# qurAI-amsterdam/SuperResolution_aniso_MRI

Measured on AMD Instinct MI355X. Metric: training slices/sec (ae_combined, 160x160, latent=128), higher is better.
Workload: dtype f32; 1 GPU; ACDC synthetic 12x(3x1x160x160) triplets, ae_combined latent=128 depth=32 scales=2, MSE synthesis loss (BASELINE configs[1]); global_batch_triplets=12, parallelism=dp1, init=reference Initializer, seed 892372, random weights, launch=captured HIP graph replay

## Files before the change

### superresolution_aniso_mri_amd/csrc/aesr_api.hip

```cpp
#include <stdarg.h>
#include <stdio.h>
#include <stdlib.h>
#include <string.h>

#include <map>
#include <mutex>
#include <tuple>

#include "../../include/aesr_hip.h"
#include "../../include/aesr_hip_dataprep.h"
#include "aesr_kernels.h"

static thread_local char g_err[512] = "";
void aesr_set_error(const char* fmt, ...) {
    va_list ap;
    va_start(ap, fmt);
    vsnprintf(g_err, sizeof(g_err), fmt, ap);
    va_end(ap);
}

static void cout_padding(int Cout, int* CoutP, int* NB) {
    if (Cout <= 16) { *CoutP = 16; *NB = 1; }
    else if (Cout <= 32) { *CoutP = 32; *NB = 2; }
    else { *CoutP = round_up(Cout, 64); *NB = 4; }
}

static bool conv_dims_ok(int N, int H, int W, int Cin, int Cout) {
    if (N < 1 || H < 1 || W < 1 || Cin < 1 || Cout < 1) return false;
    if (N > (1 << 24) || H > (1 << 15) || W > (1 << 15) || Cin > (1 << 15) || Cout > (1 << 15)) return false;
    const unsigned long long px = (unsigned long long)N * (unsigned)(H + 2) * (unsigned)(W + 2);
    return px * (unsigned long long)(Cin > Cout ? Cin : Cout) < 0x1C000000ull;
}
#define AESR_CHECK_DIMS(who, N, H, W, Cin, Cout)                                                                                            \
    do {                                                                                                                                    \
        if (!conv_dims_ok(N, H, W, Cin, Cout)) {                                                                                            \
            aesr_set_error("%s: %d x %d x %d with %d -> %d channels is empty or beyond the kernels' 32-bit element offsets (469M elements)", who, N, H, \
                           W, Cin, Cout);                                                                                                   \
            return AESR_ERR_UNSUPPORTED;                                                                                                    \
        }                                                                                                                                   \
    } while (0)

struct ConvPlan { int TI, TH, TW, NB, MBW, CinP, CoutP, NT, ksplit; };
static std::mutex g_plan_mu;

static std::map<std::tuple<int, int, int, int, int, int>, ConvPlan> g_conv_plans;

static ConvPlan plan_conv(int N, int Ho, int Wo, int Cin, int Cout, int KS) {
    std::lock_guard<std::mutex> lk(g_plan_mu);
    const auto key = std::make_tuple(N, Ho, Wo, Cin, Cout, KS);
    auto it = g_conv_plans.find(key);
    if (it != g_conv_plans.end()) return it->second;
    ConvPlan p;
    cout_padding(Cout, &p.CoutP, &p.NB);
    p.CinP = round_up(Cin, 16);
    p.MBW = (p.NB == 4) ? 2 : 4;
    const int ncout = p.CoutP / (16 * p.NB);
    int force_nt = 0;
    if (const char* e = getenv("AESR_IGEMM_NT")) force_nt = atoi(e);
    double best = 1e300;
    p.TI = 1; p.TH = 1; p.TW = 1; p.NT = 512;
// ... 58 lines not shown
}

struct WinoPlan { int TI, THt, TWt, CinP, CoutP; double cost; };
static std::map<std::tuple<int, int, int, int, int>, WinoPlan> g_wino_plans;

static WinoPlan plan_wino(int N, int H, int W, int Cin, int Cout) {
    std::lock_guard<std::mutex> lk(g_plan_mu);
    const auto key = std::make_tuple(N, H, W, Cin, Cout);
    auto it = g_wino_plans.find(key);
    if (it != g_wino_plans.end()) return it->second;
    WinoPlan p;
    p.CinP = round_up(Cin, 16);
    p.CoutP = round_up(Cout, 32);
    const int Ht = ceil_div(H, 2), Wt = ceil_div(W, 2), ncot = p.CoutP / 32, nch = p.CinP / 16;
    p.TI = 1; p.THt = 1; p.TWt = 1; p.cost = 1e300;
    auto consider = [&](int TI, int THt, int TWt) {
        const int TP = TI * THt * TWt, PP = TI * (2 * THt + 2) * (2 * TWt + 2);
        if (TP > 128 || PP * 4 > 512 * 5 || aesr_wino_lds_bytes(PP) > (size_t)160 * 1024) return;
        const long items = (long)ceil_div(N, TI) * ceil_div(Ht, THt) * ceil_div(Wt, TWt) * ncot;
        const double passes = ceil_div(ceil_div(TP, 16), 4);
        const double per = nch * (passes * 128 * 32.0 + 1200.0) + 2500.0;
        const double rounds = items <= 8 * 256 ? (double)ceil_div((int)items, 256) : (double)items / 256.0;
        const double t = per * rounds;
        if (t < p.cost * 0.999 || (t < p.cost * 1.001 && TP > p.TI * p.THt * p.TWt)) {
            if (t < p.cost) p.cost = t;
            p.TI = TI; p.THt = THt; p.TWt = TWt;
        }
    };
    for (int TI = 1; TI <= N && TI * Ht * Wt <= 128; ++TI) consider(TI, Ht, Wt);
    for (int THt = 1; THt <= Ht && THt <= 64; ++THt)
        for (int TWt = 1; TWt <= Wt && TWt <= 64; ++TWt) consider(1, THt, TWt);
    if (const char* e = getenv("AESR_WINO_TILE")) {
        int ti, th, tw;
        if (sscanf(e, "%d,%d,%d", &ti, &th, &tw) == 3) { p.TI = ti; p.THt = th < Ht ? th : Ht; p.TWt = tw < Wt ? tw : Wt; }
    }
    if (getenv("AESR_PLAN_DEBUG"))
        fprintf(stderr, "[aesr plan] wino N=%d %dx%d Cin=%d Cout=%d -> TI=%d THt=%d TWt=%d (tiles %d, patch %d px) cost %.0f\n", N, H, W, Cin, Cout,
                p.TI, p.THt, p.TWt, p.TI * p.THt * p.TWt, p.TI * (2 * p.THt + 2) * (2 * p.TWt + 2), p.cost);
    g_wino_plans[key] = p;
    return p;
}

struct WgradPlan { int variant, COT, CinP, CoutP, TH, TW, S, nslab, PWS, TWS, PSX, PSD; size_t slab_floats; };
static std::map<std::tuple<int, int, int, int, int, int>, WgradPlan> g_wgrad_plans;

static int plane_stride(int n) { return round_up(n, 64) + 4; }

static bool wgrad_wino_ok(int Cin, int Cout, int KS, int pad) {
    static int enabled = -1;
    if (enabled < 0) { const char* e = getenv("AESR_WGRAD_WINO"); enabled = (e && atoi(e) == 0) ? 0 : 1; }
    return enabled && KS == 3 && pad == 1 && Cin % 32 == 0 && Cout % 32 == 0;
}

static WgradPlan plan_wgrad_wino(int N, int H, int W, int Cin, int Cout) {
    WgradPlan p;
    p.variant = 2;
    p.COT = 32;
    p.CinP = Cin;
    p.CoutP = Cout;
    const int nchunks = (Cin / 32) * (Cout / 32);
    int S = 256 / nchunks;
    if (S >= 8) S &= ~7;
    if (S < 1) S = 1;
    double best = 1e300;
    p.TH = 16; p.TW = 8; p.S = S;
    for (int v = 0; v < 2; ++v) {
        const int TH = v ? 8 : 16, TW = v ? 16 : 8;
        const int ntiles = N * ceil_div(H, TH) * ceil_div(W, TW);
        const int s = S < ntiles ? S : ntiles;
        const double t = (double)ceil_div(ntiles, s) * (4096.0 + 1300.0);
        if (t < best) { best = t; p.TH = TH; p.TW = TW; p.S = s; }
    }
    if (const char* e = getenv("AESR_WGRAD_WINO_TILE")) {
        int th = 0, tw = 0;
        if (sscanf(e, "%d,%d", &th, &tw) == 2 && aesr_wgrad_wino_tile_ok(th, tw)) {
            p.TH = th; p.TW = tw;
            const int ntiles = N * ceil_div(H, p.TH) * ceil_div(W, p.TW);
            p.S = S < ntiles ? S : ntiles;
        }
    }
    if (const char* e = getenv("AESR_WGRAD_WINO_S")) { const int s_ = atoi(e); if (s_ > 0) p.S = s_; }
    if (const char* e = getenv("AESR_WGRAD_WINO_SMAX")) { const int s_ = atoi(e); if (s_ > 0 && p.S > s_) p.S = s_; }
    p.PWS = round_up(p.TW + 2, 4);
    p.TWS = round_up(p.TW, 4);
    p.PSX = p.PSD = 0;
    p.nslab = p.S;
    p.slab_floats = (size_t)p.nslab * 10 * p.CinP * p.CoutP;
    if (getenv("AESR_PLAN_DEBUG"))
        fprintf(stderr, "[plan_wgrad] wino N=%d %dx%d %d->%d: tile %dx%d S=%d tiles=%d\n", N, H, W, Cin, Cout, p.TH, p.TW, p.S,
                N * ceil_div(H, p.TH) * ceil_div(W, p.TW));
    return p;
}

static WgradPlan plan_wgrad(int N, int Ho, int Wo, int Cin, int Cout, int KS, int pad = -1) {
    std::lock_guard<std::mutex> lk(g_plan_mu);
    const bool wino = wgrad_wino_ok(Cin, Cout, KS, pad);
    const auto key = std::make_tuple(N, Ho, Wo, Cin, Cout, wino ? -KS : KS);
    auto it = g_wgrad_plans.find(key);
    if (it != g_wgrad_plans.end()) return it->second;
    if (wino) {
        const WgradPlan pw = plan_wgrad_wino(N, Ho, Wo, Cin, Cout);
        g_wgrad_plans[key] = pw;
        return pw;
    }
    WgradPlan p;
    p.variant = Cout > 32 ? 1 : 0;
    p.COT = p.variant ? 64 : 32;
    const int cibw = p.variant ? 2 : 1;
    p.CinP = round_up(Cin, 32);
    p.CoutP = round_up(Cout, p.COT);
    const size_t max_lds = 52 * 1024;
    const int nchunks = (p.CinP / 32) * (p.CoutP / p.COT);
    const int S0 = round_up(768 / nchunks > 0 ? 768 / nchunks : 1, 8);
    double best = 1e300;
    p.TH = 1; p.TW = 8; p.S = 1;
    for (int TW = 8; TW <= 64; TW += 8) {
        if (TW - 8 >= Wo) break;
        for (int TH = 1; TH <= 32 && TH <= Ho; ++TH) {
            const int PH = TH + KS - 1, PWp = TW + KS - 1, PWS = PWp + (PWp & 1);
            if (PH * PWp * 8 > 256 * (p.variant ? 4 : 6) || TH * TW * (p.COT / 4) > 256 * (p.variant ? 5 : 6)) break;
            const size_t ldsb = ((size_t)32 * plane_stride(PH * PWS) + (size_t)p.COT * plane_stride(TH * TW)) * 4;
            if (ldsb > max_lds) break;
            const int ntiles = N * ceil_div(Ho, TH) * ceil_div(Wo, TW);
            const int S = S0 < ntiles ? S0 : ntiles;
            const double rounds = (double)ceil_div(ntiles, S);
            const double mf = 3.0 * (TH * TW / 8) * (2 * KS * KS * cibw) * 32.0;
            const double t = rounds * (mf + 4500.0);
            if (t < best) { best = t; p.TH = TH; p.TW = TW; p.S = S; }
        }
    }
    if (const char* e = getenv("AESR_WGRAD_TILE")) {
        int th = 0, tw = 0;
        if (sscanf(e, "%d,%d", &th, &tw) == 2 && th > 0 && tw > 0 && tw % 8 == 0) {
            p.TH = th < Ho ? th : Ho; p.TW = tw;
            const int ntiles = N * ceil_div(Ho, p.TH) * ceil_div(Wo, p.TW);
            p.S = S0 < ntiles ? S0 : ntiles;
        }
    }
    if (const char* e = getenv("AESR_WGRAD_S")) {
        const int s_ = atoi(e);
        const int ntiles = N * ceil_div(Ho, p.TH) * ceil_div(Wo, p.TW);
        if (s_ > 0) p.S = s_ < ntiles ? s_ : ntiles;
    }
// ... 354 lines not shown
    AESR_CHECK_ARG(!x_up2 || (wgrad_wino_ok(Cin, Cout, KS, pad) && !((H | W) & 1)), "aesr_conv2d_wgrad_partial: the folded upsampling needs "
                   "the Winograd weight-gradient kernel (3x3, padding 1, Cin, Cout multiples of 32) and an even size");
    return wgrad_impl(x, dy, nullptr, nullptr, workspace, N, H, W, Cin, Cout, KS, pad, stream, x_up2);
}

int aesr_conv2d_wgrad_reduce_many(const aesr_wgrad_reduce_job* jobs_host, int njobs, void* stream) {
    AESR_CHECK_ARG(jobs_host && njobs > 0, "aesr_conv2d_wgrad_reduce_many: no jobs");
    for (int j0 = 0; j0 < njobs; j0 += REDUCE_MAX_JOBS) {
        ReduceTable t;
        memset(&t, 0, sizeof(t));
        t.njobs = njobs - j0 < REDUCE_MAX_JOBS ? njobs - j0 : REDUCE_MAX_JOBS;
        int nb = 0;
        for (int k = 0; k < t.njobs; ++k) {
            const aesr_wgrad_reduce_job& jb = jobs_host[j0 + k];
            AESR_CHECK_ARG(jb.workspace && jb.dw && jb.N > 0 && (jb.KS == 1 || jb.KS == 3), "aesr_conv2d_wgrad_reduce_many: bad job %d", j0 + k);
            AESR_CHECK_ARG(conv_dims_ok(jb.N, jb.H, jb.W, jb.Cin, jb.Cout) && jb.pad >= 0 && jb.pad < jb.KS && jb.H + 2 * jb.pad >= jb.KS && jb.W + 2 * jb.pad >= jb.KS,
                           "aesr_conv2d_wgrad_reduce_many: job %d: bad shape", j0 + k);
            const int Ho = jb.H + 2 * jb.pad - jb.KS + 1, Wo = jb.W + 2 * jb.pad - jb.KS + 1;
            const WgradPlan p = plan_wgrad(jb.N, Ho, Wo, jb.Cin, jb.Cout, jb.KS, jb.pad);
            ReduceJob& o = t.job[k];
            o.slab = jb.workspace; o.dw = jb.dw; o.db = jb.db; o.nslab = p.nslab; o.KS2 = jb.KS * jb.KS; o.Cin = jb.Cin; o.CinP = p.CinP;
            o.Cout = jb.Cout; o.CoutP = p.CoutP; o.block0 = nb;
            nb += ceil_div(o.KS2 * jb.Cin * jb.Cout + (jb.db ? jb.Cout : 0), 64);
        }
        t.nblocks = nb;
        if (int e = aesr_launch_wgrad_reduce_many(t, (hipStream_t)stream)) return e;
    }
    return AESR_OK;
}

int aesr_conv2d_wgrad_up2_supported(int Cin, int Cout) { return wgrad_wino_ok(Cin, Cout, 3, 1) ? 1 : 0; }

int aesr_conv2d_wgrad_up2(const float* x_half, const float* dy, float* dw, float* db, float* workspace, int N, int H, int W, int Cin,
                          int Cout, void* stream) {
    AESR_CHECK_ARG(wgrad_wino_ok(Cin, Cout, 3, 1) && !((H | W) & 1), "aesr_conv2d_wgrad_up2: needs the Winograd weight-gradient kernel "
                   "(Cin, Cout multiples of 32; got %d -> %d) and an even size", Cin, Cout);
    return wgrad_impl(x_half, dy, dw, db, workspace, N, H, W, Cin, Cout, 3, 1, stream, 1);
}

static int wgrad_impl(const float* x, const float* dy, float* dw, float* db, float* workspace, int N, int H, int W, int Cin,
                      int Cout, int KS, int pad, void* stream, int x_up2) {
    AESR_CHECK_ARG(x && dy && workspace && N > 0, "aesr_conv2d_wgrad: null pointer or empty shape");
    AESR_CHECK_ARG(Cin % 4 == 0 && Cout % 4 == 0, "aesr_conv2d_wgrad: Cin=%d, Cout=%d must be multiples of 4", Cin, Cout);
    AESR_CHECK_ARG((KS == 1 || KS == 3) && pad >= 0 && pad < KS, "aesr_conv2d_wgrad: unsupported KS=%d pad=%d", KS, pad);
    AESR_CHECK_DIMS("aesr_conv2d_wgrad", N, H, W, Cin, Cout);
    const int Ho = H + 2 * pad - KS + 1, Wo = W + 2 * pad - KS + 1;
    AESR_CHECK_ARG(Ho > 0 && Wo > 0, "aesr_conv2d_wgrad: the %d x %d input is smaller than the %d x %d filter", H, W, KS, KS);
    const WgradPlan p = plan_wgrad(N, Ho, Wo, Cin, Cout, KS, pad);
    WgradArgs a;
    a.x = x; a.dy = dy; a.slab = workspace;
    a.N = N; a.H = H; a.W = W; a.Cin = Cin; a.CinP = p.CinP; a.Cout = Cout; a.CoutP = p.CoutP; a.Ho = Ho; a.Wo = Wo; a.pad = pad;
    a.TH = p.TH; a.TW = p.TW; a.tiles_y = ceil_div(Ho, p.TH); a.tiles_x = ceil_div(Wo, p.TW);
    a.ntiles = N * a.tiles_y * a.tiles_x; a.S = p.S;
    a.PWS = p.PWS; a.TWS = p.TWS; a.PSX = p.PSX; a.PSD = p.PSD; a.dbgbuf = nullptr; a.x_up2 = x_up2;
    if (p.variant == 2) {
        if (int e = aesr_launch_conv_wgrad_wino(a, (hipStream_t)stream)) return e;
    } else if (int e = aesr_launch_conv_wgrad(a, KS, p.variant, (hipStream_t)stream)) {
        return e;
    }
    if (!dw) return AESR_OK;
    return aesr_launch_wgrad_reduce(workspace, dw, db, p.nslab, KS, Cin, p.CinP, Cout, p.CoutP, (hipStream_t)stream);
}

int aesr_conv2d_smallcin_fwd(const float* in, const float* w, const float* bias, const float* y_saved, float* out, int N,
                             int H, int W, int Cin, int Cout, int KS, int pad, int act, int mask_act, float slope,
                             int transpose, int bcast, const float* ca_host, const float* cb_host, void* stream) {
    AESR_CHECK_ARG(in && w && out && N > 0 && Cin >= 1 && Cin <= 4 && Cout > 0, "aesr_conv2d_smallcin_fwd: need 1 <= Cin <= 4");
    AESR_CHECK_ARG(!bcast || (ca_host && cb_host), "aesr_conv2d_smallcin_fwd: bcast needs ca/cb");
    SmallArgs a;
    memset(&a, 0, sizeof(a));
    a.in = in; a.w = w; a.bias = bias; a.ysave = y_saved; a.out = out;
    a.N = N; a.H = H; a.W = W; a.Cin = Cin; a.Cout = Cout; a.KS = KS; a.pad = pad;
    a.Ho = H + 2 * pad - KS + 1; a.Wo = W + 2 * pad - KS + 1;
    a.act = act; a.mask_act = mask_act; a.slope = slope; a.transpose = transpose; a.bcast = bcast;
    for (int i = 0; i < Cin && bcast; ++i) { a.ca[i] = ca_host[i]; a.cb[i] = cb_host[i]; }
    return aesr_launch_smallcin_fwd(a, (hipStream_t)stream);
}

int aesr_conv2d_smallcin_dgrad(const float* dy, const float* w, float* dx, int N, int H, int W, int Cin, int Cout, int KS,
                               int pad, int bcast, const float* ca_host, void* stream) {
    AESR_CHECK_ARG(dy && w && dx && N > 0 && Cin >= 1 && Cin <= 4 && Cout > 0, "aesr_conv2d_smallcin_dgrad: need 1 <= Cin <= 4");
    AESR_CHECK_ARG(!bcast || ca_host, "aesr_conv2d_smallcin_dgrad: bcast needs ca");
    SmallDgradArgs a;
    memset(&a, 0, sizeof(a));
    a.dy = dy; a.w = w; a.dx = dx; a.N = N; a.H = H; a.W = W; a.Cin = Cin; a.Cout = Cout; a.KS = KS; a.pad = pad; a.bcast = bcast;
    a.Ho = H + 2 * pad - KS + 1; a.Wo = W + 2 * pad - KS + 1;
    for (int i = 0; i < Cin && bcast; ++i) a.ca[i] = ca_host[i];
    return aesr_launch_smallcin_dgrad(a, (hipStream_t)stream);
}

#define SMALL_WGRAD_NWG 512
size_t aesr_small_wgrad_workspace_floats(int nout) { return (size_t)SMALL_WGRAD_NWG * nout; }

int aesr_conv2d_smallcin_wgrad(const float* in, const float* dout, float* dw, float* db, float* workspace, int N, int H,
                               int W, int Cin, int Cout, int pad, void* stream) {
    AESR_CHECK_ARG(in && dout && dw && db && workspace && Cin >= 1 && Cin <= 4, "aesr_conv2d_smallcin_wgrad: need 1 <= Cin <= 4");
    AESR_CHECK_ARG(Cout >= 4 && Cout % 4 == 0 && 256 % (Cout / 4) == 0 && Cout <= 256,
                   "aesr_conv2d_smallcin_wgrad: Cout=%d must be a multiple of 4 with Cout/4 dividing 256", Cout);
    SmallWgradArgs a;
    a.in = in; a.dout = dout; a.partial = workspace; a.N = N; a.H = H; a.W = W; a.Cin = Cin; a.Cout = Cout; a.pad = pad;
    a.Ho = H + 2 * pad; a.Wo = W + 2 * pad;
    if (int e = aesr_launch_smallcin_wgrad(a, SMALL_WGRAD_NWG, (hipStream_t)stream)) return e;
    return aesr_launch_sum_partials(workspace, SMALL_WGRAD_NWG, Cout * (Cin + 1), dw, Cout * Cin, db, (hipStream_t)stream);
}

int aesr_conv2d_cout1_fwd(const float* x, const float* w, const float* bias, float* out, int N, int H, int W, int Cin, int act,
                          float slope, void* stream) {
// ... 556 lines not shown
```

### superresolution_aniso_mri_amd/csrc/aesr_kernels.h

```cpp
#pragma once
#include "aesr_common.h"

struct IgemmArgs {
    const float* in; const float* wpk; const float* bias; const float* ysave; float* out;
    int N, H, W, Cin, CinP, Cout, CoutP, Ho, Wo, pad;
    int TI, TH, TW, tiles_y, tiles_x, nitems, dbg;
    int NT;
    int ksplit;
    float* dbgbuf;
    int act, mask_act;
    float slope;
};
int aesr_launch_conv_igemm(const IgemmArgs& a, int KS, int NB, int MBW, hipStream_t st);
int aesr_launch_conv_ksplit_fixup(const float* partial, const float* bias, const float* ysave, float* out, size_t nelem, int Cout,
                                  int ksplit, int act, int mask_act, float slope, hipStream_t st);
int aesr_launch_pack_weights(const float* w, float* p, int Cout, int Cin, int KS, int KinP, int NoutP, int TN, int transpose, hipStream_t st);

struct WinoArgs {
    const float* in; const float* upk; const float* bias; const float* ysave; float* out;
    int N, H, W, Cin, CinP, Cout, CoutP;
    int TI, THt, TWt;
    int regs_y, regs_x, nitems;
    unsigned m_ncot, m_regs_x, m_regs_y;
    int act, mask_act;
    float slope;
    float* dbgbuf;
    int flags;
    int in_up2;
    int out_sum2;
    int bpi, nblk;
    unsigned m_bpi;
    int nw, rowP, imgP, patch_fl, sw_a, sw_m, sw_b;
    int xcd_map;
    double plan_cost;
    int nfull, tail_k;
    int ksplit, kchunks, split_bytes;
    unsigned m_ksplit;
    float* ws;
    size_t ws_floats;
    const float* post_scale; const float* post_shift;
    int post_pool;
};
int aesr_launch_conv_wino(const WinoArgs& a, hipStream_t st);
bool aesr_wino_res_ok(const WinoArgs& a);
int aesr_launch_conv_wino_res(const WinoArgs& a, hipStream_t st);
int aesr_wino_ring_mode();
bool aesr_wino_ring_takes(const WinoArgs& a);
int aesr_launch_conv_wino_ring(const WinoArgs& a, hipStream_t st);
size_t aesr_wino_ring_workspace_floats(const WinoArgs& a);
unsigned aesr_wino_ring_timeouts();
size_t aesr_wino_lds_bytes(int patch_pixels);

#define PACK_MAX_JOBS 32
struct PackJob { const float* w; float* p; int Cout, Cin, KS, KinP, NoutP, TN, transpose, block0; };
struct PackTable { int njobs, nblocks; PackJob job[PACK_MAX_JOBS]; };
int aesr_launch_pack_many(const PackTable& t, hipStream_t st);
enum { PREP_PACK = 0, PREP_WINO_PACK = 1, PREP_STEM_FOLD = 2, PREP_COUT1_FLIP = 3 };
struct PrepJob { const float* w; const float* aux0; const float* aux1; float* out; int kind, Cout, Cin, KS, KinP, NoutP, TN, transpose, block0; };
struct PrepTable { int njobs, nblocks; PrepJob job[PACK_MAX_JOBS]; };
int aesr_launch_prep_many(const PrepTable& t, hipStream_t st);
int aesr_launch_wino_pack_many(const PackTable& t, hipStream_t st);

struct WgradArgs {
    const float* x; const float* dy; float* slab;
    int N, H, W, Cin, CinP, Cout, CoutP, Ho, Wo, pad;
    int TH, TW, tiles_y, tiles_x, ntiles;
    int S;
    int PWS, TWS, PSX, PSD;
    float* dbgbuf;
    int x_up2;
};
int aesr_launch_conv_wgrad(const WgradArgs& a, int KS, int variant, hipStream_t st);
int aesr_launch_conv_wgrad_wino(const WgradArgs& a, hipStream_t st);
size_t aesr_wgrad_wino_lds_bytes(int TH, int TW);
bool aesr_wgrad_wino_tile_ok(int TH, int TW);
#define REDUCE_MAX_JOBS 16
struct ReduceJob { const float* slab; float* dw; float* db; int nslab, KS2, Cin, CinP, Cout, CoutP, block0; };
struct ReduceTable { int njobs, nblocks; ReduceJob job[REDUCE_MAX_JOBS]; };
int aesr_launch_wgrad_reduce_many(const ReduceTable& t, hipStream_t st);
int aesr_launch_wgrad_reduce(const float* slab, float* dw, float* db, int nslab, int KS, int Cin, int CinP, int Cout, int CoutP, hipStream_t st);

struct SmallArgs {
    const float* in; const float* w; const float* bias; const float* ysave; float* out;
    int N, H, W, Cin, Cout, Ho, Wo, KS, pad;
    int act, mask_act;
    float slope;
    int transpose, bcast;
    float ca[4], cb[4];
};
struct SmallDgradArgs {
    const float* dy; const float* w; float* dx;
    int N, H, W, Cin, Cout, Ho, Wo, KS, pad, bcast;
    float ca[4];
};
struct SmallWgradArgs {
    const float* in; const float* dout; float* partial;
    int N, H, W, Cin, Cout, Ho, Wo, pad;
};
struct Cout1WgradArgs {
    const float* x; const float* dy; float* partial;
    int N, H, W, Cin, TH, TW, tiles_y, tiles_x, ntiles;
};
struct Cout1FwdArgs {
    const float* x; const float* w; const float* bias; float* out;
    int N, H, W, Cin, TH, TW, tiles_y, tiles_x, act;
    float slope;
};
int aesr_launch_cout1_fwd(const Cout1FwdArgs& a, hipStream_t st);
int aesr_launch_smallcin_fwd(const SmallArgs& a, hipStream_t st);
int aesr_launch_smallcin_dgrad(const SmallDgradArgs& a, hipStream_t st);
int aesr_launch_sum_partials(const float* partial, int np, int n, float* out0, int n0, float* out1, hipStream_t st);
int aesr_launch_smallcin_wgrad(const SmallWgradArgs& a, int nwg, hipStream_t st);
int aesr_launch_cout1_wgrad(const Cout1WgradArgs& a, int nwg, hipStream_t st);

struct ThinArgs {
    const float* s;
    const float* w;
    const float* be;
    const float* b;
    const float* ysave;
    float* out;
    const float* t;
    float* partial;
    int N, Hs, Ws, Ho, Wo, C, ps;
    int act, mask_act;
    float slope;
    int with_be;
    int tiles_y, tiles_x, ntiles;
// ... 103 lines not shown
```

### superresolution_aniso_mri_amd/csrc/conv_wgrad_wino.hip

```cpp
#include <stdio.h>
#include <stdlib.h>

#include <type_traits>
#include <utility>

#include "aesr_kernels.h"

constexpr int WW_OOB = 0x70000000;
typedef float f32x2 __attribute__((ext_vector_type(2)));
#ifndef WW_ABL
#define WW_ABL 0
#endif

template <int... I, class F>
__device__ __forceinline__ void ww_for(std::integer_sequence<int, I...>, F&& f) {
    (f(std::integral_constant<int, I>{}), ...);
}
template <int N, class F>
__device__ __forceinline__ void ww_rep(F&& f) { ww_for(std::make_integer_sequence<int, N>{}, f); }

__device__ __forceinline__ void ww_dma(__amdgpu_buffer_rsrc_t rs, float* lds_wave_base, int byte_off) {
    __builtin_amdgcn_raw_ptr_buffer_load_lds(rs, (__attribute__((address_space(3))) void*)lds_wave_base, 16, byte_off, 0, 0, 0);
}

#define WW_PK(dst, a, b, mods)                                                          \
    do {                                                                                \
        f32x2& d_ = dst;                                                                \
        const f32x2 a_ = a, b_ = b;                                                     \
        asm volatile("v_pk_add_f32 %0, %1, %2 " mods : "=v"(d_) : "v"(a_), "v"(b_));    \
    } while (0)
#define WW_M_ADD ""
#define WW_M_SUB "neg_lo:[0,1] neg_hi:[0,1]"
#define WW_M_T01 "op_sel:[0,0] op_sel_hi:[1,0] neg_lo:[0,1] neg_hi:[0,0]"
#define WW_M_T23 "op_sel:[1,0] op_sel_hi:[1,1] neg_lo:[1,0] neg_hi:[0,1]"
#define WW_M_LL "op_sel:[0,0] op_sel_hi:[0,0] neg_lo:[0,0] neg_hi:[0,1]"
#define WW_M_HH "op_sel:[1,1] op_sel_hi:[1,1] neg_lo:[0,0] neg_hi:[0,1]"
#define WW_M_SELF "op_sel:[0,1] op_sel_hi:[0,1] neg_lo:[0,0] neg_hi:[0,1]"

struct WwTile {
    int n, ty, tx;
};

template <int TH, int TW, bool STAMP>
__global__ __launch_bounds__(256, 1) void conv_wgrad_wino_f32(WgradArgs a) {
    constexpr int CIT = 32, COT = 32;
    static_assert((TH == 16 && TW == 8) || (TH == 8 && TW == 16), "tiles: 8 k-steps, rows of whole 8-pixel DMA segments");
    constexpr int PH = TH + 2, PWL = TW == 8 ? 16 : 32, TWL = TW;
    constexpr int XFL = PH * PWL * 32, DFL = TH * TWL * 32;
    constexpr int KPR = TW >> 3;
    constexpr int SPR = PWL / 8, SPRD = TW / 8;
    constexpr int NXS = PH * SPR / 4, NDS = TH * SPRD / 4;
    constexpr int RXS = 4 / SPR, RDS = 4 / SPRD;
    static_assert(2 * (XFL + DFL) * 4 <= 160 * 1024 && (PH * SPR) % 4 == 0 && (TH * SPRD) % 4 == 0, "LDS / segment split");

    extern __shared__ __attribute__((aligned(16))) float lds[];
    const int tid = threadIdx.x, lane = tid & 63;
    const int wave = __builtin_amdgcn_readfirstlane(tid >> 6);
    const int l15 = lane & 15, g = lane >> 4;
    const int nci = a.CinP / CIT, nchunks = nci * (a.CoutP / COT);
    int chunk, split;
    if ((a.S & 7) == 0) {
        const int xcd = blockIdx.x & 7, local = blockIdx.x >> 3;
        chunk = local % nchunks;
        split = (local / nchunks) * 8 + xcd;
    } else {
        chunk = blockIdx.x % nchunks;
        split = blockIdx.x / nchunks;
    }
    const int ciy = chunk % nci, coz = chunk / nci;
    const int ci0 = ciy * CIT, co0 = coz * COT;
    float* const ldsX0 = lds;
    float* const ldsD0 = lds + 2 * XFL;
    const bool do_bias = ciy == 0;

    const int sh = a.x_up2 ? 1 : 0;
    const int xH = a.H >> sh, xW = a.W >> sh;
    const int ximg = xH * xW * a.Cin * 4, dimg = a.H * a.W * a.Cout * 4;
    const int xrow = xW * a.Cin * 4, drow = a.W * a.Cout * 4;
    const int sgx = wave % SPR, rx0 = wave / SPR, sgd = wave % SPRD, rd0 = wave / SPRD;
    const int pxl = lane >> 3, pos = lane & 7;
    const int quad = pos ^ (((pxl >> 1) & 1) << 2);
    const int pcx = 8 * sgx + pxl, pcd = 8 * sgd + pxl;
    const int lcx = (((pcx - sh) >> sh) * a.Cin + ci0 + 4 * quad) * 4;
    const int lcd = (pcd * a.Cout + co0 + 4 * quad) * 4;
    const int tpi = a.tiles_y * a.tiles_x;
    const int dS_n = a.S / tpi, dS_r = a.S - dS_n * tpi, dS_ty = dS_r / a.tiles_x, dS_tx = dS_r - dS_ty * a.tiles_x;
    auto advance = [&](WwTile t) {
        t.tx += dS_tx;
        if (t.tx >= a.tiles_x) { t.tx -= a.tiles_x; ++t.ty; }
        t.ty += dS_ty;
        if (t.ty >= a.tiles_y) { t.ty -= a.tiles_y; ++t.n; }
        t.n += dS_n;
        return t;
    };
    auto fetch = [&](const WwTile& t, int buf) {
        const bool valid = t.n < a.N;
// ... 62 lines not shown
                         : "=&v"(p0_), "=&v"(p1_) : "v"(ad), "n"(0), "n"(PWL / 2), "n"(PWL), "n"(3 * PWL / 2) : "memory");
        });
        ww_rep<4>([&](auto Kc) {
            constexpr int o = decltype(Kc)::value >> 1, e = decltype(Kc)::value & 1;
            const unsigned ad = ld[o][e] + (unsigned)(du * 4);
            f32x2& y_ = Mp[nb][o][e];
            asm volatile("ds_read2st64_b32 %0, %1 offset0:0 offset1:%2" : "=&v"(y_) : "v"(ad), "n"(TWL / 2) : "memory");
        });
    };
    auto op_transform = [&](int nb) {
        asm volatile("s_waitcnt lgkmcnt(0)" ::: "memory");
        ww_rep<2>([&](auto Ic) {
            constexpr int i = decltype(Ic)::value;
            f32x2 T[2][4];
            ww_rep<4>([&](auto Cc) {
                constexpr int c = decltype(Cc)::value;
                WW_PK(T[0][c], P[i][c][0], P[i][c][1], WW_M_T01);
                WW_PK(T[1][c], P[i][c][0], P[i][c][1], WW_M_T23);
            });
            ww_rep<2>([&](auto Sc) {
                constexpr int s_ = decltype(Sc)::value;
                WW_PK(Vp[nb][i][s_][0], T[s_][0], T[s_][2], WW_M_SUB);
                WW_PK(Vp[nb][i][s_][1], T[s_][1], T[s_][2], WW_M_ADD);
                WW_PK(Vp[nb][i][s_][2], T[s_][2], T[s_][1], WW_M_SUB);
                WW_PK(Vp[nb][i][s_][3], T[s_][1], T[s_][3], WW_M_SUB);
            });
        });
        ww_rep<2>([&](auto Oc) {
            constexpr int o = decltype(Oc)::value;
            WW_PK(Mp[nb][o][2], Mp[nb][o][0], Mp[nb][o][0], WW_M_SELF);
            WW_PK(Mp[nb][o][3], Mp[nb][o][1], Mp[nb][o][1], WW_M_SELF);
            WW_PK(Mp[nb][o][4], Mp[nb][o][0], Mp[nb][o][1], WW_M_LL);
            WW_PK(Mp[nb][o][7], Mp[nb][o][0], Mp[nb][o][1], WW_M_HH);
            WW_PK(Mp[nb][o][5], Mp[nb][o][2], Mp[nb][o][3], WW_M_LL);
            WW_PK(Mp[nb][o][6], Mp[nb][o][2], Mp[nb][o][3], WW_M_HH);
            accb[o] += Mp[nb][o][5][0];
        });
    };
    auto mfmas = [&](auto Q0c, auto Nc, int cb) {
        ww_rep<decltype(Nc)::value>([&](auto Dc) {
            constexpr int q = decltype(Q0c)::value + decltype(Dc)::value, x = q >> 2, i = (q >> 1) & 1, o = q & 1;
            constexpr int r = x >> 2, k = x & 3;
            constexpr int mi = k == 0 ? (r == 0 || r == 3 ? 0 : 2) : k == 3 ? (r == 0 || r == 3 ? 1 : 3) : 4 + r;
            constexpr int mh = k == 0 || k == 3 ? (r >= 2 ? 1 : 0) : k - 1;
            f32x4& acc_ = acc[x][i][o];
            const float va_ = Vp[cb][i][r >> 1][k][r & 1], vb_ = Mp[cb][o][mi][mh];
            asm volatile("v_mfma_f32_16x16x4_f32 %0, %1, %2, %0" : "+a"(acc_) : "v"(va_), "v"(vb_));
        });
    };
    auto step_xu = [&](int j, int buf) { const int ks = wave + 4 * j, tyl = ks / KPR, kx = ks - tyl * KPR; return buf * XFL + ((2 * tyl) * PWL + 8 * kx) * 32; };
    auto step_du = [&](int j, int buf) { const int ks = wave + 4 * j, tyl = ks / KPR, kx = ks - tyl * KPR; return buf * DFL + ((2 * tyl) * TWL + 8 * kx) * 32; };
    using C0 = std::integral_constant<int, 0>;
    using C16 = std::integral_constant<int, 16>;
    using C32 = std::integral_constant<int, 32>;

    long long tph[3] = {0, 0, 0}, tq = 0;
#define WW_STAMP(k)                                                   \
    if constexpr (STAMP) {                                            \
        const long long t_ = (long long)__builtin_amdgcn_s_memtime(); \
        tph[k] += t_ - tq;                                            \
        tq = t_;                                                      \
    }
    if constexpr (STAMP) tq = (long long)__builtin_amdgcn_s_memtime();

    WwTile t0, t1, t2;
    {
        t0.n = split / tpi;
        const int rem = split - t0.n * tpi;
        t0.ty = rem / a.tiles_x;
        t0.tx = rem - t0.ty * a.tiles_x;
        if (split >= a.ntiles) t0.n = a.N;
    }
    t1 = advance(t0);
    t2 = advance(t1);
    fetch(t0, 0);
    fetch(t1, 1);
    asm volatile("s_waitcnt vmcnt(0)" ::: "memory");
    __syncthreads();
    int buf = 0;
    op_read(step_xu(0, 0), step_du(0, 0), 0);
    op_transform(0);
    WW_STAMP(2)
    if (t0.n < a.N) do {
        __builtin_amdgcn_sched_barrier(0);
#if WW_ABL != 3 && WW_ABL != 4
        op_read(step_xu(1, buf), step_du(1, buf), 1);
#endif
        mfmas(C0{}, C16{}, 0);
#if WW_ABL != 2 && WW_ABL != 4
        op_transform(1);
#endif
        mfmas(C16{}, std::integral_constant<int, 48>{}, 0);
        __builtin_amdgcn_sched_barrier(0);
        WW_STAMP(0)
        asm volatile("s_waitcnt vmcnt(0) lgkmcnt(0)" ::: "memory");
        __syncthreads();
        WW_STAMP(1)
        __builtin_amdgcn_sched_barrier(0);
#if WW_ABL != 3 && WW_ABL != 4
        op_read(step_xu(0, buf ^ 1), step_du(0, buf ^ 1), 0);
#endif
        mfmas(C0{}, C16{}, 1);
        __builtin_amdgcn_sched_barrier(0);
#if WW_ABL != 1 && WW_ABL != 4
        fetch(t2, buf);
#endif
        __builtin_amdgcn_sched_barrier(0);
        mfmas(C16{}, C16{}, 1);
#if WW_ABL != 2 && WW_ABL != 4
        op_transform(0);
#endif
        mfmas(C32{}, C32{}, 1);
        __builtin_amdgcn_sched_barrier(0);
        t0 = t1;
        t1 = t2;
        t2 = advance(t2);
        buf ^= 1;
    } while (t0.n < a.N);
    WW_STAMP(0)
    asm volatile("s_waitcnt vmcnt(0) lgkmcnt(0)" ::: "memory");
    __syncthreads();
    if (STAMP && lane == 0)
        for (int k = 0; k < 3; ++k) a.dbgbuf[(blockIdx.x * 4 + wave) * 3 + k] = (float)tph[k];

    f32x4 dg[9][2][2];
#pragma unroll
    for (int i = 0; i < 2; ++i)
#pragma unroll
        for (int o = 0; o < 2; ++o) {
            f32x4 R[3][4];
#pragma unroll
            for (int j = 0; j < 4; ++j) {
                const f32x4 u0_ = acc[0 + j][i][o], u1 = acc[4 + j][i][o], u2 = acc[8 + j][i][o], u3 = -acc[12 + j][i][o];
                const f32x4 s = j == 3 ? (f32x4){-1.f, -1.f, -1.f, -1.f} : (f32x4){1.f, 1.f, 1.f, 1.f};
                R[0][j] = s * (u0_ + 0.5f * (u1 + u2));
                R[1][j] = s * (0.5f * (u1 - u2));
                R[2][j] = s * (0.5f * (u1 + u2) + u3);
            }
#pragma unroll
            for (int r = 0; r < 3; ++r) {
                dg[r * 3 + 0][i][o] = R[r][0] + 0.5f * (R[r][1] + R[r][2]);
                dg[r * 3 + 1][i][o] = 0.5f * (R[r][1] - R[r][2]);
                dg[r * 3 + 2][i][o] = 0.5f * (R[r][1] + R[r][2]) + R[r][3];
            }
        }
#pragma unroll
    for (int o = 0; o < 2; ++o) {
        accb[o] += __shfl_xor(accb[o], 16, 64);
        accb[o] += __shfl_xor(accb[o], 32, 64);
    }
    f32x4* ex = (f32x4*)lds;
    float* exb = lds + 4 * 36 * 64 * 4;
#pragma unroll
    for (int t = 0; t < 9; ++t)
#pragma unroll
        for (int i = 0; i < 2; ++i)
#pragma unroll
            for (int o = 0; o < 2; ++o) ex[(wave * 36 + (t * 4 + i * 2 + o)) * 64 + lane] = dg[t][i][o];
    if (g == 0) {
        exb[wave * 32 + l15] = accb[0];
        exb[wave * 32 + 16 + l15] = accb[1];
    }
    __syncthreads();
    const size_t plane = (size_t)a.CinP * a.CoutP;
    float* sl = a.slab + (size_t)split * 10 * plane;
#pragma unroll
    for (int q = 0; q < 9; ++q) {
        const int blk = wave * 9 + q;
        const int t = blk >> 2, i = (blk >> 1) & 1, o = blk & 1;
        f32x4 v = ex[(0 * 36 + blk) * 64 + lane];
#pragma unroll
        for (int w = 1; w < 4; ++w) v += ex[(w * 36 + blk) * 64 + lane];
        const int co = co0 + o * 16 + l15;
#pragma unroll
        for (int e = 0; e < 4; ++e) {
            const int ci = ci0 + i * 16 + g * 4 + e;
            sl[t * plane + (size_t)ci * a.CoutP + co] = v[e];
        }
    }
    if (wave == 0 && do_bias && g == 0) {
#pragma unroll
        for (int o = 0; o < 2; ++o) {
            float bsum = exb[0 * 32 + o * 16 + l15];
#pragma unroll
            for (int w = 1; w < 4; ++w) bsum += exb[w * 32 + o * 16 + l15];
            sl[9 * plane + co0 + o * 16 + l15] = bsum;
        }
    }
}

size_t aesr_wgrad_wino_lds_bytes(int TH, int TW) {
    const size_t xfl = (size_t)(TH + 2) * (TW == 8 ? 16 : 32) * 32, dfl = (size_t)TH * TW * 32;
    const size_t bufs = 2 * (xfl + dfl) * sizeof(float);
    const size_t exch = ((size_t)4 * 36 * 64 * 4 + 4 * 32) * sizeof(float);
    return bufs > exch ? bufs : exch;
}

bool aesr_wgrad_wino_tile_ok(int TH, int TW) { return (TH == 16 && TW == 8) || (TH == 8 && TW == 16); }

template <int TH, int TW>
static int launch_wgrad_wino(const WgradArgs& a, hipStream_t st) {
    const size_t shmem = aesr_wgrad_wino_lds_bytes(TH, TW);
    static bool attr_set[AESR_MAX_DEVICES] = {};
    int dev_ = 0;
    if (hipGetDevice(&dev_) != hipSuccess || dev_ < 0 || dev_ >= AESR_MAX_DEVICES) dev_ = 0;
    if (!attr_set[dev_]) {
        const hipError_t e_ = hipFuncSetAttribute((const void*)conv_wgrad_wino_f32<TH, TW, false>, hipFuncAttributeMaxDynamicSharedMemorySize, 160 * 1024);
        if (e_ == hipSuccess) (void)hipFuncSetAttribute((const void*)conv_wgrad_wino_f32<TH, TW, true>, hipFuncAttributeMaxDynamicSharedMemorySize, 160 * 1024);
        if (e_ != hipSuccess) {
            aesr_set_error("conv_wgrad_wino_f32: hipFuncSetAttribute(MaxDynamicSharedMemorySize = 160 KB) failed: %s", hipGetErrorString(e_));
            return AESR_ERR_HIP;
        }
        attr_set[dev_] = true;
    }
    dim3 grid(a.S * (a.CinP / 32) * (a.CoutP / 32));
    if (getenv("AESR_WGRAD_WINO_DBG") && grid.x <= 4096) {
        static float* dbuf = nullptr;
        if (!dbuf) (void)hipMalloc(&dbuf, 4096 * 4 * 3 * sizeof(float));
        WgradArgs b = a;
        b.dbgbuf = dbuf;
        hipLaunchKernelGGL((conv_wgrad_wino_f32<TH, TW, true>), grid, dim3(256), shmem, st, b);
        (void)hipStreamSynchronize(st);
        static float host[4096 * 4 * 3];
        (void)hipMemcpy(host, dbuf, (size_t)grid.x * 4 * 3 * sizeof(float), hipMemcpyDeviceToHost);
        double s3[3] = {0, 0, 0};
        for (unsigned i = 0; i < grid.x * 4; ++i) for (int k = 0; k < 3; ++k) s3[k] += host[i * 3 + k];
        const double visits = (double)((a.ntiles + a.S - 1) / a.S);
        const int nks = (TH >> 1) * (TW >> 3);
        fprintf(stderr, "[wgrad-wino stamps] grid=%u tile %dx%d S=%d (%.0f visits, %d k-steps = %d MFMA cycles per wave and visit) per visit, cycles: "
                "k-step loop %.0f | barrier %.0f || fill %.0f\n", grid.x, TH, TW, a.S, visits, nks, nks / 4 * 64 * 32,
                s3[0] / grid.x / 4 / visits, s3[1] / grid.x / 4 / visits, s3[2] / grid.x / 4);
        return AESR_OK;
    }
    hipLaunchKernelGGL((conv_wgrad_wino_f32<TH, TW, false>), grid, dim3(256), shmem, st, a);
    AESR_LAUNCH_CHECK("conv_wgrad_wino_f32");
    return AESR_OK;
}

int aesr_launch_conv_wgrad_wino(const WgradArgs& a, hipStream_t st) {
    if ((size_t)a.H * a.W * a.Cin * 4 >= (size_t)0x10000000 || (size_t)a.H * a.W * a.Cout * 4 >= (size_t)0x10000000) {
        aesr_set_error("conv_wgrad_wino: images of 256 MB or more need 64-bit lane offsets (not built)");
        return AESR_ERR_UNSUPPORTED;
    }
    if (a.x_up2 && ((a.H | a.W) & 1)) {
        aesr_set_error("conv_wgrad_wino: the folded Upsample(x2) needs even convolution sizes (got %dx%d)", a.H, a.W);
        return AESR_ERR_ARG;
    }
    if (!aesr_wgrad_wino_tile_ok(a.TH, a.TW) || a.pad != 1 || a.Ho != a.H || a.Wo != a.W) {
        aesr_set_error("conv_wgrad_wino: tile %dx%d is not 16x8 or 8x16 (or not 3x3 / padding 1)", a.TH, a.TW);
        return AESR_ERR_ARG;
    }
    if (a.CinP % 32 != 0 || a.CoutP % 32 != 0 || a.Cin != a.CinP || a.Cout != a.CoutP || a.S < 1 || a.S > a.ntiles ||
        a.tiles_y != ceil_div(a.H, a.TH) || a.tiles_x != ceil_div(a.W, a.TW) || a.ntiles != a.N * a.tiles_y * a.tiles_x) {
        aesr_set_error("conv_wgrad_wino: channel counts must be multiples of 32 and the tile grid consistent (S=%d, %d tiles)", a.S, a.ntiles);
        return AESR_ERR_ARG;
    }
    if (a.TH == 16) return launch_wgrad_wino<16, 8>(a, st);
    return launch_wgrad_wino<8, 16>(a, st);
}
```

Baseline: 15380 slices/s.

## Skip MFMA work for half-empty last tile row in Winograd wgrad

When the last row of tiles covers only half a tile or less of the image (and there are at most 4 tile rows), a new SHORT kernel variant branches over the second half of the MFMA k-steps for that row. Those steps would only multiply padding. The planner's cost model now charges such short visits less and balances per-slab cost, which can change the chosen tile shape and split. In the SHORT variant, full tiles lose the interleaving of MFMAs with the operand reads, fetch and transform, so they may run slower. The kernel's debug timestamps are extended to report full and short visits separately.

```diff
diff --git a/superresolution_aniso_mri_amd/csrc/aesr_api.hip b/superresolution_aniso_mri_amd/csrc/aesr_api.hip
--- a/superresolution_aniso_mri_amd/csrc/aesr_api.hip
+++ b/superresolution_aniso_mri_amd/csrc/aesr_api.hip
@@ -3,9 +3,11 @@
 #include <stdlib.h>
 #include <string.h>
 
+#include <algorithm>
 #include <map>
 #include <mutex>
 #include <tuple>
+#include <vector>
 
 #include "../../include/aesr_hip.h"
 #include "../../include/aesr_hip_dataprep.h"
@@ -170,6 +172,8 @@
     return enabled && KS == 3 && pad == 1 && Cin % 32 == 0 && Cout % 32 == 0;
 }
 
+static const double WGRAD_WINO_SHORT_VISIT = 0.69;
+
 static WgradPlan plan_wgrad_wino(int N, int H, int W, int Cin, int Cout) {
     WgradPlan p;
     p.variant = 2;
@@ -186,7 +190,11 @@
         const int TH = v ? 8 : 16, TW = v ? 16 : 8;
         const int ntiles = N * ceil_div(H, TH) * ceil_div(W, TW);
         const int s = S < ntiles ? S : ntiles;
-        const double t = (double)ceil_div(ntiles, s) * (4096.0 + 1300.0);
+        const double full_visit = 4096.0 + 1300.0, short_visit = WGRAD_WINO_SHORT_VISIT * full_visit;
+        const int tiles_x = ceil_div(W, TW), tpi = ceil_div(H, TH) * tiles_x, short_ty = aesr_wgrad_wino_short_row(H, TH, 1);
+        std::vector<double> cost((size_t)s, 0.0);
+        for (int i = 0; i < ntiles; ++i) cost[i % s] += (i % tpi) / tiles_x == short_ty ? short_visit : full_visit;
+        const double t = *std::max_element(cost.begin(), cost.end());
         if (t < best) { best = t; p.TH = TH; p.TW = TW; p.S = s; }
     }
     if (const char* e = getenv("AESR_WGRAD_WINO_TILE")) {
@@ -205,8 +213,8 @@
     p.nslab = p.S;
     p.slab_floats = (size_t)p.nslab * 10 * p.CinP * p.CoutP;
     if (getenv("AESR_PLAN_DEBUG"))
-        fprintf(stderr, "[plan_wgrad] wino N=%d %dx%d %d->%d: tile %dx%d S=%d tiles=%d\n", N, H, W, Cin, Cout, p.TH, p.TW, p.S,
-                N * ceil_div(H, p.TH) * ceil_div(W, p.TW));
+        fprintf(stderr, "[plan_wgrad] wino N=%d %dx%d %d->%d: tile %dx%d S=%d tiles=%d short=%d\n", N, H, W, Cin, Cout, p.TH, p.TW, p.S,
+                N * ceil_div(H, p.TH) * ceil_div(W, p.TW), aesr_wgrad_wino_short_row(H, p.TH, 1) >= 0 ? N * ceil_div(W, p.TW) : 0);
     return p;
 }
 
@@ -667,7 +675,7 @@
     a.N = N; a.H = H; a.W = W; a.Cin = Cin; a.CinP = p.CinP; a.Cout = Cout; a.CoutP = p.CoutP; a.Ho = Ho; a.Wo = Wo; a.pad = pad;
     a.TH = p.TH; a.TW = p.TW; a.tiles_y = ceil_div(Ho, p.TH); a.tiles_x = ceil_div(Wo, p.TW);
     a.ntiles = N * a.tiles_y * a.tiles_x; a.S = p.S;
-    a.PWS = p.PWS; a.TWS = p.TWS; a.PSX = p.PSX; a.PSD = p.PSD; a.dbgbuf = nullptr; a.x_up2 = x_up2;
+    a.PWS = p.PWS; a.TWS = p.TWS; a.PSX = p.PSX; a.PSD = p.PSD; a.dbgbuf = nullptr; a.x_up2 = x_up2; a.short_ty = -1;
     if (p.variant == 2) {
         if (int e = aesr_launch_conv_wgrad_wino(a, (hipStream_t)stream)) return e;
     } else if (int e = aesr_launch_conv_wgrad(a, KS, p.variant, (hipStream_t)stream)) {
diff --git a/superresolution_aniso_mri_amd/csrc/aesr_kernels.h b/superresolution_aniso_mri_amd/csrc/aesr_kernels.h
--- a/superresolution_aniso_mri_amd/csrc/aesr_kernels.h
+++ b/superresolution_aniso_mri_amd/csrc/aesr_kernels.h
@@ -69,11 +69,13 @@
     int PWS, TWS, PSX, PSD;
     float* dbgbuf;
     int x_up2;
+    int short_ty;
 };
 int aesr_launch_conv_wgrad(const WgradArgs& a, int KS, int variant, hipStream_t st);
 int aesr_launch_conv_wgrad_wino(const WgradArgs& a, hipStream_t st);
 size_t aesr_wgrad_wino_lds_bytes(int TH, int TW);
 bool aesr_wgrad_wino_tile_ok(int TH, int TW);
+int aesr_wgrad_wino_short_row(int H, int TH, int mode);
 #define REDUCE_MAX_JOBS 16
 struct ReduceJob { const float* slab; float* dw; float* db; int nslab, KS2, Cin, CinP, Cout, CoutP, block0; };
 struct ReduceTable { int njobs, nblocks; ReduceJob job[REDUCE_MAX_JOBS]; };
diff --git a/superresolution_aniso_mri_amd/csrc/conv_wgrad_wino.hip b/superresolution_aniso_mri_amd/csrc/conv_wgrad_wino.hip
--- a/superresolution_aniso_mri_amd/csrc/conv_wgrad_wino.hip
+++ b/superresolution_aniso_mri_amd/csrc/conv_wgrad_wino.hip
@@ -37,11 +37,18 @@
 #define WW_M_HH "op_sel:[1,1] op_sel_hi:[1,1] neg_lo:[0,0] neg_hi:[0,1]"
 #define WW_M_SELF "op_sel:[0,1] op_sel_hi:[0,1] neg_lo:[0,0] neg_hi:[0,1]"
 
+#define WW_SKIP_IF_EQ(a, b)                                                                                \
+    do {                                                                                                   \
+        const int a_ = a, b_ = b;                                                                          \
+        asm volatile("s_cmp_eq_u32 %0, %1\n\ts_cbranch_scc1 1f" : : "s"(a_), "s"(b_) : "scc", "memory");    \
+    } while (0)
+#define WW_SKIP_END() asm volatile("1:" ::: "memory")
+
 struct WwTile {
     int n, ty, tx;
 };
 
-template <int TH, int TW, bool STAMP>
+template <int TH, int TW, bool STAMP, bool SHORT>
 __global__ __launch_bounds__(256, 1) void conv_wgrad_wino_f32(WgradArgs a) {
     constexpr int CIT = 32, COT = 32;
     static_assert((TH == 16 && TW == 8) || (TH == 8 && TW == 16), "tiles: 8 k-steps, rows of whole 8-pixel DMA segments");
@@ -210,9 +217,8 @@
     auto step_du = [&](int j, int buf) { const int ks = wave + 4 * j, tyl = ks / KPR, kx = ks - tyl * KPR; return buf * DFL + ((2 * tyl) * TWL + 8 * kx) * 32; };
     using C0 = std::integral_constant<int, 0>;
     using C16 = std::integral_constant<int, 16>;
-    using C32 = std::integral_constant<int, 32>;
-
-    long long tph[3] = {0, 0, 0}, tq = 0;
+
+    long long tph[5] = {0, 0, 0, 0, 0}, tq = 0;
 #define WW_STAMP(k)                                                   \
     if constexpr (STAMP) {                                            \
         const long long t_ = (long long)__builtin_amdgcn_s_memtime(); \
@@ -250,36 +256,57 @@
 #endif
         mfmas(C16{}, std::integral_constant<int, 48>{}, 0);
         __builtin_amdgcn_sched_barrier(0);
-        WW_STAMP(0)
+        if constexpr (STAMP) { if (t0.ty != a.short_ty) { WW_STAMP(0) } else { WW_STAMP(3) } }
         asm volatile("s_waitcnt vmcnt(0) lgkmcnt(0)" ::: "memory");
         __syncthreads();
-        WW_STAMP(1)
-        __builtin_amdgcn_sched_barrier(0);
+        if constexpr (STAMP) { if (t0.ty != a.short_ty) { WW_STAMP(1) } else { WW_STAMP(4) } }
+        if constexpr (!SHORT) {
+            __builtin_amdgcn_sched_barrier(0);
 #if WW_ABL != 3 && WW_ABL != 4
-        op_read(step_xu(0, buf ^ 1), step_du(0, buf ^ 1), 0);
-#endif
-        mfmas(C0{}, C16{}, 1);
-        __builtin_amdgcn_sched_barrier(0);
+            op_read(step_xu(0, buf ^ 1), step_du(0, buf ^ 1), 0);
+#endif
+            mfmas(C0{}, C16{}, 1);
+            __builtin_amdgcn_sched_barrier(0);
 #if WW_ABL != 1 && WW_ABL != 4
-        fetch(t2, buf);
-#endif
-        __builtin_amdgcn_sched_barrier(0);
-        mfmas(C16{}, C16{}, 1);
+            fetch(t2, buf);
+#endif
+            __builtin_amdgcn_sched_barrier(0);
+            mfmas(C16{}, C16{}, 1);
 #if WW_ABL != 2 && WW_ABL != 4
-        op_transform(0);
-#endif
-        mfmas(C32{}, C32{}, 1);
-        __builtin_amdgcn_sched_barrier(0);
+            op_transform(0);
+#endif
+            mfmas(std::integral_constant<int, 32>{}, std::integral_constant<int, 32>{}, 1);
+            __builtin_amdgcn_sched_barrier(0);
+        } else {
+            __builtin_amdgcn_sched_barrier(0);
+#if WW_ABL != 3 && WW_ABL != 4
+            op_read(step_xu(0, buf ^ 1), step_du(0, buf ^ 1), 0);
+#endif
+            __builtin_amdgcn_sched_barrier(0);
+#if WW_ABL != 1 && WW_ABL != 4
+            fetch(t2, buf);
+#endif
+            __builtin_amdgcn_sched_barrier(0);
+            WW_SKIP_IF_EQ(t0.ty, a.short_ty);
+            mfmas(C0{}, std::integral_constant<int, 64>{}, 1);
+            WW_SKIP_END();
+            __builtin_amdgcn_sched_barrier(0);
+#if WW_ABL != 2 && WW_ABL != 4
+            op_transform(0);
+#endif
+            __builtin_amdgcn_sched_barrier(0);
+        }
+        if constexpr (STAMP) { if (t0.ty != a.short_ty) { WW_STAMP(0) } else { WW_STAMP(3) } }
         t0 = t1;
         t1 = t2;
         t2 = advance(t2);
         buf ^= 1;
     } while (t0.n < a.N);
-    WW_STAMP(0)
+    WW_STAMP(2)
     asm volatile("s_waitcnt vmcnt(0) lgkmcnt(0)" ::: "memory");
     __syncthreads();
     if (STAMP && lane == 0)
-        for (int k = 0; k < 3; ++k) a.dbgbuf[(blockIdx.x * 4 + wave) * 3 + k] = (float)tph[k];
+        for (int k = 0; k < 5; ++k) a.dbgbuf[(blockIdx.x * 4 + wave) * 5 + k] = (float)tph[k];
 
     f32x4 dg[9][2][2];
 #pragma unroll
@@ -356,6 +383,12 @@
 
 bool aesr_wgrad_wino_tile_ok(int TH, int TW) { return (TH == 16 && TW == 8) || (TH == 8 && TW == 16); }
 
+int aesr_wgrad_wino_short_row(int H, int TH, int mode) {
+    const int tiles_y = (H + TH - 1) / TH;
+    if (mode <= 0 || H - (tiles_y - 1) * TH > TH / 2) return -1;
+    return mode >= 2 || tiles_y <= 4 ? tiles_y - 1 : -1;
+}
+
 template <int TH, int TW>
 static int launch_wgrad_wino(const WgradArgs& a, hipStream_t st) {
     const size_t shmem = aesr_wgrad_wino_lds_bytes(TH, TW);
@@ -363,8 +396,10 @@
     int dev_ = 0;
     if (hipGetDevice(&dev_) != hipSuccess || dev_ < 0 || dev_ >= AESR_MAX_DEVICES) dev_ = 0;
     if (!attr_set[dev_]) {
-        const hipError_t e_ = hipFuncSetAttribute((const void*)conv_wgrad_wino_f32<TH, TW, false>, hipFuncAttributeMaxDynamicSharedMemorySize, 160 * 1024);
-        if (e_ == hipSuccess) (void)hipFuncSetAttribute((const void*)conv_wgrad_wino_f32<TH, TW, true>, hipFuncAttributeMaxDynamicSharedMemorySize, 160 * 1024);
+        hipError_t e_ = hipFuncSetAttribute((const void*)conv_wgrad_wino_f32<TH, TW, false, false>, hipFuncAttributeMaxDynamicSharedMemorySize, 160 * 1024);
+        if (e_ == hipSuccess) e_ = hipFuncSetAttribute((const void*)conv_wgrad_wino_f32<TH, TW, false, true>, hipFuncAttributeMaxDynamicSharedMemorySize, 160 * 1024);
+        if (e_ == hipSuccess) (void)hipFuncSetAttribute((const void*)conv_wgrad_wino_f32<TH, TW, true, false>, hipFuncAttributeMaxDynamicSharedMemorySize, 160 * 1024);
+        if (e_ == hipSuccess) (void)hipFuncSetAttribute((const void*)conv_wgrad_wino_f32<TH, TW, true, true>, hipFuncAttributeMaxDynamicSharedMemorySize, 160 * 1024);
         if (e_ != hipSuccess) {
             aesr_set_error("conv_wgrad_wino_f32: hipFuncSetAttribute(MaxDynamicSharedMemorySize = 160 KB) failed: %s", hipGetErrorString(e_));
             return AESR_ERR_HIP;
@@ -374,28 +409,35 @@
     dim3 grid(a.S * (a.CinP / 32) * (a.CoutP / 32));
     if (getenv("AESR_WGRAD_WINO_DBG") && grid.x <= 4096) {
         static float* dbuf = nullptr;
-        if (!dbuf) (void)hipMalloc(&dbuf, 4096 * 4 * 3 * sizeof(float));
+        if (!dbuf) (void)hipMalloc(&dbuf, 4096 * 4 * 5 * sizeof(float));
         WgradArgs b = a;
         b.dbgbuf = dbuf;
-        hipLaunchKernelGGL((conv_wgrad_wino_f32<TH, TW, true>), grid, dim3(256), shmem, st, b);
+        if (a.short_ty >= 0) hipLaunchKernelGGL((conv_wgrad_wino_f32<TH, TW, true, true>), grid, dim3(256), shmem, st, b);
+        else hipLaunchKernelGGL((conv_wgrad_wino_f32<TH, TW, true, false>), grid, dim3(256), shmem, st, b);
         (void)hipStreamSynchronize(st);
-        static float host[4096 * 4 * 3];
-        (void)hipMemcpy(host, dbuf, (size_t)grid.x * 4 * 3 * sizeof(float), hipMemcpyDeviceToHost);
-        double s3[3] = {0, 0, 0};
-        for (unsigned i = 0; i < grid.x * 4; ++i) for (int k = 0; k < 3; ++k) s3[k] += host[i * 3 + k];
-        const double visits = (double)((a.ntiles + a.S - 1) / a.S);
+        static float host[4096 * 4 * 5];
+        (void)hipMemcpy(host, dbuf, (size_t)grid.x * 4 * 5 * sizeof(float), hipMemcpyDeviceToHost);
+        double s5[5] = {0, 0, 0, 0, 0};
+        for (unsigned i = 0; i < grid.x * 4; ++i) for (int k = 0; k < 5; ++k) s5[k] += host[i * 5 + k];
+        const int nshort = a.short_ty >= 0 ? a.N * a.tiles_x : 0, nfull = a.ntiles - nshort;
+        const double wv = 4.0 * (a.CinP / 32) * (a.CoutP / 32);
+        const double dfull = wv * (nfull > 0 ? nfull : 1), dshort = wv * (nshort > 0 ? nshort : 1);
         const int nks = (TH >> 1) * (TW >> 3);
-        fprintf(stderr, "[wgrad-wino stamps] grid=%u tile %dx%d S=%d (%.0f visits, %d k-steps = %d MFMA cycles per wave and visit) per visit, cycles: "
-                "k-step loop %.0f | barrier %.0f || fill %.0f\n", grid.x, TH, TW, a.S, visits, nks, nks / 4 * 64 * 32,
-                s3[0] / grid.x / 4 / visits, s3[1] / grid.x / 4 / visits, s3[2] / grid.x / 4);
+        fprintf(stderr, "[wgrad-wino stamps] grid=%u tile %dx%d S=%d (%d full + %d short visits per chunk, %d k-steps = %d MFMA cycles per wave and full "
+                "visit) per visit, cycles: full: k-step loop %.0f | barrier %.0f || short: k-step loop %.0f | barrier %.0f || fill %.0f\n", grid.x, TH,
+                TW, a.S, nfull, nshort, nks, nks / 4 * 64 * 32, s5[0] / dfull, s5[1] / dfull, s5[3] / dshort, s5[4] / dshort, s5[2] / grid.x / 4);
         return AESR_OK;
     }
-    hipLaunchKernelGGL((conv_wgrad_wino_f32<TH, TW, false>), grid, dim3(256), shmem, st, a);
+    if (a.short_ty >= 0) hipLaunchKernelGGL((conv_wgrad_wino_f32<TH, TW, false, true>), grid, dim3(256), shmem, st, a);
+    else hipLaunchKernelGGL((conv_wgrad_wino_f32<TH, TW, false, false>), grid, dim3(256), shmem, st, a);
     AESR_LAUNCH_CHECK("conv_wgrad_wino_f32");
     return AESR_OK;
 }
 
-int aesr_launch_conv_wgrad_wino(const WgradArgs& a, hipStream_t st) {
+int aesr_launch_conv_wgrad_wino(const WgradArgs& a_in, hipStream_t st) {
+    WgradArgs a = a_in;
+    const char* se = getenv("AESR_WGRAD_WINO_SHORT");
+    a.short_ty = aesr_wgrad_wino_tile_ok(a.TH, a.TW) ? aesr_wgrad_wino_short_row(a.H, a.TH, se ? atoi(se) : 1) : -1;
     if ((size_t)a.H * a.W * a.Cin * 4 >= (size_t)0x10000000 || (size_t)a.H * a.W * a.Cout * 4 >= (size_t)0x10000000) {
         aesr_set_error("conv_wgrad_wino: images of 256 MB or more need 64-bit lane offsets (not built)");
         return AESR_ERR_UNSUPPORTED;
```

Result: no change. 15720 slices/s (median of 6 runs) (+2.3%).
